# 10258392511/InverseProblemWithDiffusionModel

Measured on AMD Instinct MI355X. Metric: ALD reconstructions/sec (128x128 complex, R=40, 4-coil), higher is better.
Workload: dtype f32 (convolutions: operands as two fp16 pieces = 22 significand bits + 2 signs, three fp16 MFMAs per product, fp32 accumulate; every image scaled into fp16's range by an exact power of two from its producer's per-image maxima: any fp32 input, DESIGN.md 4.2); 1 GPU; ACDC-style 128x128 complex SENSE R=40 4-coil ALD reconstruction, NCSNv2Deepest ngf=128 (94.1M params, seeded random init), sigma 348->0.01 x 2311 levels x 3 steps, L2Penalty, denoise; 14 posterior samples = 14 on rank 0 + 13 per further rank (the 105-sample / 8-GPU partition of BASELINE config 3); samples_total=14, samples_this_rank=14, parallelism=sample-sharded x1, hip_graph=True, state_finite=True

## Files before the change

include/ipdm.h:

```cpp
#ifndef IPDM_H
#define IPDM_H

#include <stddef.h>
#include <stdint.h>

#ifdef __cplusplus
extern "C" {
#endif

#define IPDM_OK 0
#define IPDM_EINVAL (-1)
#define IPDM_EUNSUPPORTED (-2)

#define IPDM_ACT_NONE 0
#define IPDM_ACT_ELU 1
#define IPDM_ACT_RELU 2
#define IPDM_ACT_LRELU02 3
#define IPDM_ACT_SWISH 4
#define IPDM_ACT_COPY 5

#define IPDM_AMAX_WAYS 8
#define IPDM_AMAX_SLOT 128

#define IPDM_ABI_VERSION 4
// ... 192 lines not shown

int ipdm_philox_normal_f32(float* out, uint64_t seed, int64_t sample_offset, int64_t step_id, int plane,
                           int64_t n_samples, int64_t sample_elems, void* stream);

int ipdm_philox_block_host(uint64_t seed, int64_t sample, int64_t step_id, int plane, uint32_t quad, uint32_t* out4);


int ipdm_instnorm_plus_coef_f32(const float* x, const float* alpha, const float* gamma, const float* beta,
                                float* coef, int B, int C, int HW,
                                float* amax_bound ,
                                void* stream);
int ipdm_cond_instnorm_plus_coef_f32(const float* x, const float* embed, const int64_t* labels, int num_classes, int bias,
                                     float* coef, int B, int C, int HW, float* amax_bound, void* stream);
int ipdm_affine_act_f32(const float* x, const float* coef, float* y, int B, int C, int HW, int act, void* stream);
int ipdm_act_f32(const float* x, float* y, int64_t n, int act, void* stream);
int ipdm_scale_shift_f32(const float* x, float* y, int64_t n, float a, float b, void* stream);
int ipdm_add_f32(const float* x, const float* y, float* out, int64_t n, void* stream);
int ipdm_div_sigma_f32(const float* x, const float* sigmas, const int64_t* labels, float* out,
                       int B, int64_t sample_elems, void* stream);
int ipdm_conv3x3_thin_supported(int Cin, int Cout, int H, int W);
int ipdm_conv3x3_thin_f32(const float* x, const float* w, const float* bias,
                          const float* coef ,
                          float* out, int B, int Cin, int Cout, int H, int W, void* stream);
int ipdm_maxpool5_f32(const float* x, float* y, int planes, int H, int W, void* stream);
int ipdm_affine_avgpool5_f32(const float* x, const float* coef, float* y, int planes, int H, int W, void* stream);
int ipdm_meanpool2_f32(const float* x, float* y, int planes, int H, int W, void* stream);
int ipdm_bilinear_f32(const float* x, float* out, int planes, int in_h, int in_w, int out_h, int out_w,
                      int accumulate, int act ,
                      int planes_per_image, float* amax_out ,
                      void* stream);
int ipdm_trilinear_f32(const float* x, float* out, int planes, int in_d, int in_h, int in_w, int out_d, int out_h,
                       int out_w, int accumulate, int act, int planes_per_image, float* amax_out, void* stream);

int ipdm_groupnorm_coef_f32(const float* x, const float* weight, const float* bias, float* coef,
                            int B, int C, int HW, int G, float eps,
                            float* plane_amax ,
                            void* stream);
int ipdm_groupnorm_coef_partials_f32(const float* part1, int C1, const float* part2, int C2, int P, const float* weight,
                                     const float* bias, float* coef , int B, int G, float eps, void* stream);
int ipdm_groupnorm_coef_cat_f32(const float* x1, int C1, const float* x2, int C2, const float* weight, const float* bias,
                                float* coef, int B, int HW, int G, float eps, float* plane_amax ,
                                void* stream);
int ipdm_affine_act_cat_f32(const float* x1, int C1, const float* x2, int C2, const float* coef, float* y, int B, int HW,
                            int act, void* stream);
int ipdm_linear_f32(const float* x, const float* W, const float* bias, float* y, int B, int In, int Out,
                    int act, void* stream);
// ... 165 lines not shown
```

inverseproblemwithdiffusionmodel_amd/_lib.py:

```python
import ctypes
import os

import torch
from ctypes import c_char_p, c_double, c_float, c_int, c_int64, c_uint64, c_void_p


class ConvExt(ctypes.Structure):
    _fields_ = [("in_amax", c_void_p), ("bias_bstride", c_int), ("out_scale", c_float), ("res_second", c_int),
                ("out_amax", c_void_p), ("act_amax", c_void_p)]


_HERE = os.path.dirname(os.path.abspath(__file__))
LIB_PATH = os.environ.get("IPDM_LIB") or os.path.join(_HERE, "libipdm.so")

P = c_void_p

SIGNATURES = {
    "ipdm_abi_version": [],
    "ipdm_build_arch": [],
    "ipdm_upfirdn2d_f32": [P, P, P] + [c_int] * 14 + [P],
    "ipdm_fused_bias_act_f32": [P, P, P, P, c_int64, c_int, c_int, c_int, c_int, c_float, c_float, P],
    "ipdm_upfirdn2d_f16": [P, P, P] + [c_int] * 14 + [P],
    "ipdm_upfirdn2d_f64": [P, P, P] + [c_int] * 14 + [P],
    "ipdm_fused_bias_act_f16": [P, P, P, P, c_int64, c_int, c_int, c_int, c_int, c_float, c_float, P],
# ... 54 lines not shown
    "ipdm_espirit_kernels_c64": [P, c_int, c_int, c_int, c_double, P, P, P, P, P, P, c_int, c_int, c_int, c_int, P],
    "ipdm_espirit_pixel_c64": [P, P, c_int, c_float, c_int, P, P, c_int, c_int, c_int, c_int, P],
    "ipdm_espirit_c64": [P, c_int, c_int, c_int, c_double, c_float, c_int, P, P, P, P, P, P, P, c_int, c_int, c_int, c_int, P],
    "ipdm_kspace_tavg_c64": [P, P, c_int, P, P, c_int, c_int, c_int, c_int, c_int, P],
    "ipdm_singlecoil_prox_f32": [P, P, P, P, c_int, c_float, c_int, P, P, P, c_int, c_int, c_int, P],
    "ipdm_ald_singlecoil_step_f32": [P, P, P, P, P, P, c_float, c_float, c_uint64, c_int64, c_int64, P,
                                     P, P, c_int, c_float, c_int, P, c_int, c_int, c_int, P],
    "ipdm_langevin_step_f32": [P, P, P, c_float, c_float, c_uint64, c_int64, c_int64, P, c_int64, c_int64, P],
    "ipdm_philox_normal_f32": [P, c_uint64, c_int64, c_int64, c_int, c_int64, c_int64, P],
    "ipdm_philox_block_host": [c_uint64, c_int64, c_int64, c_int, ctypes.c_uint32, P],
    "ipdm_instnorm_plus_coef_f32": [P, P, P, P, P, c_int, c_int, c_int, P, P],
    "ipdm_cond_instnorm_plus_coef_f32": [P, P, P, c_int, c_int, P, c_int, c_int, c_int, P, P],
    "ipdm_affine_act_f32": [P, P, P, c_int, c_int, c_int, c_int, P],
    "ipdm_act_f32": [P, P, c_int64, c_int, P],
    "ipdm_scale_shift_f32": [P, P, c_int64, c_float, c_float, P],
    "ipdm_add_f32": [P, P, P, c_int64, P],
    "ipdm_div_sigma_f32": [P, P, P, P, c_int, c_int64, P],
    "ipdm_maxpool5_f32": [P, P, c_int, c_int, c_int, P],
    "ipdm_affine_avgpool5_f32": [P, P, P, c_int, c_int, c_int, P],
    "ipdm_meanpool2_f32": [P, P, c_int, c_int, c_int, P],
    "ipdm_bilinear_f32": [P, P, c_int, c_int, c_int, c_int, c_int, c_int, c_int, c_int, P, P],
    "ipdm_conv3x3_thin_supported": [c_int, c_int, c_int, c_int],
    "ipdm_conv3x3_thin_f32": [P, P, P, P, P, c_int, c_int, c_int, c_int, c_int, P],
    "ipdm_trilinear_f32": [P, P, c_int, c_int, c_int, c_int, c_int, c_int, c_int, c_int, c_int, c_int, P, P],
    "ipdm_groupnorm_coef_f32": [P, P, P, P, c_int, c_int, c_int, c_int, c_float, P, P],
    "ipdm_groupnorm_coef_partials_f32": [P, c_int, P, c_int, c_int, P, P, P, c_int, c_int, c_float, P],
    "ipdm_groupnorm_coef_cat_f32": [P, c_int, P, c_int, P, P, P, c_int, c_int, c_int, c_float, P, P],
    "ipdm_affine_act_cat_f32": [P, c_int, P, c_int, P, P, c_int, c_int, c_int, P],
    "ipdm_linear_f32": [P, P, P, P, c_int, c_int, c_int, c_int, P],
    "ipdm_attention_f32": [P, P, P, P, c_int, c_int, c_int, c_float, P],
    "ipdm_axpby_f32": [P, P, P, c_int64, c_float, c_float, P],
    "ipdm_sample_axpy2_f32": [P, P, P, P, P, P, c_int, c_int64, P],
    "ipdm_sample_norm_f32": [P, P, c_int, c_int64, P],
    "ipdm_conv_pack_weight_f32": [P, P, c_int, c_int, c_int, P],
    "ipdm_conv2d_f32": [P, P, P, P, c_int, P, P, P, c_int] + [c_int] * 8 + [P],
    "ipdm_conv_wino_weight_f32": [P, P, c_int, c_int, P],
    "ipdm_conv2d_wino_supported": [c_int, c_int, c_int, c_int, c_int],
    "ipdm_conv2d_wino_f32": [P, P, P, P, P, P, c_int, c_int, c_int, c_int, c_int, c_int, c_int, P],
    "ipdm_debug_set_stamp_buffer": [P],
    "ipdm_debug_lds_optin_count": [],
    "ipdm_conv3d_f32": [P, P, P, P, c_int, P, P, P, c_int] + [c_int] * 8 + [P],
    "ipdm_maxpool3d5_f32": [P, P, c_int, c_int, c_int, c_int, P],
    "ipdm_temporal_taps_f32": [P, P, c_int, c_int, c_int, c_int, c_int, P],
    "ipdm_conv_bx3_weight_bytes": [c_int, c_int, c_int],
    "ipdm_conv_bx3_pack_weight": [P, P, c_int, c_int, c_int, P],
    "ipdm_conv2d_bx3_f32": [P, P, P, P, c_int, P, P, P, c_int] + [c_int] * 7 + [P, P],
# ... 105 lines not shown
```

inverseproblemwithdiffusionmodel_amd/csrc/conv_thin.hip:

```cpp
#include "ipdm_common.h"

namespace {

template <int CIN>
__global__ __launch_bounds__(256) void conv3x3_fewin_kernel(const float* __restrict__ x, const float* __restrict__ w,
                                                            const float* __restrict__ bias, const float* __restrict__ coef,
                                                            float* __restrict__ out, int B, int Cout, int H, int W,
                                                            int co_blk) {
  const int Q = W >> 2;
  const long long items = (long long)B * H * Q;
  const int co0 = blockIdx.y * co_blk;
  const int co1 = min(Cout, co0 + co_blk);
  for (long long it = (long long)blockIdx.x * 256 + threadIdx.x; it < items; it += (long long)gridDim.x * 256) {
    const int q = (int)(it % Q);
    const long long t = it / Q;
    const int y = (int)(t % H);
    const int b = (int)(t / H);
    float in[CIN][3][6];
#pragma unroll
    for (int ci = 0; ci < CIN; ++ci) {
      float c0 = 0.f, c1 = 1.f, c2 = 0.f;
      if (coef) {
        const float* cf = coef + ((long long)b * CIN + ci) * 3;
        c0 = cf[0]; c1 = cf[1]; c2 = cf[2];
      }
#pragma unroll
      for (int r = 0; r < 3; ++r) {
        const int yy = y + r - 1;
        const bool row_ok = yy >= 0 && yy < H;
        const float* rp = x + (((long long)b * CIN + ci) * H + (row_ok ? yy : 0)) * W + 4 * q;
        const float4 m = *reinterpret_cast<const float4*>(rp);
        const float l = rp[q > 0 ? -1 : 0], rr = rp[q < Q - 1 ? 4 : 3];
        in[ci][r][0] = (row_ok && q > 0) ? (l - c0) * c1 + c2 : 0.f;
        in[ci][r][1] = row_ok ? (m.x - c0) * c1 + c2 : 0.f;
        in[ci][r][2] = row_ok ? (m.y - c0) * c1 + c2 : 0.f;
        in[ci][r][3] = row_ok ? (m.z - c0) * c1 + c2 : 0.f;
        in[ci][r][4] = row_ok ? (m.w - c0) * c1 + c2 : 0.f;
        in[ci][r][5] = (row_ok && q < Q - 1) ? (rr - c0) * c1 + c2 : 0.f;
      }
    }
    float* op = out + (((long long)b * Cout + co0) * H + y) * W + 4 * q;
    for (int co = co0; co < co1; ++co, op += (long long)H * W) {
      const float* wp = w + (long long)co * CIN * 9;
      const float bv = bias ? bias[co] : 0.f;
      float a0 = bv, a1 = bv, a2 = bv, a3 = bv;
#pragma unroll
      for (int ci = 0; ci < CIN; ++ci)
#pragma unroll
        for (int r = 0; r < 3; ++r)
#pragma unroll
          for (int c = 0; c < 3; ++c) {
            const float wv = wp[(ci * 3 + r) * 3 + c];
            a0 = fmaf(wv, in[ci][r][c], a0);
            a1 = fmaf(wv, in[ci][r][c + 1], a1);
            a2 = fmaf(wv, in[ci][r][c + 2], a2);
            a3 = fmaf(wv, in[ci][r][c + 3], a3);
          }
      *reinterpret_cast<float4*>(op) = make_float4(a0, a1, a2, a3);
    }
  }
}

template <int COUT, bool SHFL>
__global__ __launch_bounds__(256) void conv3x3_fewout_kernel(const float* __restrict__ x, const float* __restrict__ w,
                                                             const float* __restrict__ bias, float* __restrict__ out,
                                                             int B, int Cin, int H, int W) {
  __shared__ float red[3][COUT][4][64];
  const int Q = W >> 2;
  const long long items = (long long)B * H * Q;
  const long long HW = (long long)H * W;
  const int lane = threadIdx.x & 63, grp = threadIdx.x >> 6;
  for (long long it0 = (long long)blockIdx.x * 64; it0 < items; it0 += (long long)gridDim.x * 64) {
    const long long it = it0 + lane < items ? it0 + lane : items - 1;
    const bool live = it0 + lane < items;
    const int q = (int)(it % Q);
    const long long t = it / Q;
    const int y = (int)(t % H);
    const int b = (int)(t / H);
    float acc[COUT][3][4], hl[COUT][3], hr[COUT][3];
#pragma unroll
    for (int co = 0; co < COUT; ++co)
// ... 66 lines not shown
        for (int j = 0; j < 4; ++j) red[grp - 1][co][j][lane] = o[co][j];
    }
    __syncthreads();
    if (grp == 0 && live) {
#pragma unroll
      for (int co = 0; co < COUT; ++co) {
        const float bv = bias ? bias[co] : 0.f;
        float v[4];
#pragma unroll
        for (int j = 0; j < 4; ++j) v[j] = bv + (((o[co][j] + red[0][co][j][lane]) + red[1][co][j][lane]) + red[2][co][j][lane]);
        *reinterpret_cast<float4*>(out + (((long long)b * COUT + co) * H + y) * W + 4 * q) = make_float4(v[0], v[1], v[2], v[3]);
      }
    }
    __syncthreads();
  }
}

}

extern "C" int ipdm_conv3x3_thin_supported(int Cin, int Cout, int H, int W) {
  return (W % 4 == 0 && H > 0 && ((Cin >= 1 && Cin <= 3 && Cout >= 1) || (Cout >= 1 && Cout <= 3 && Cin >= 1))) ? 1 : 0;
}

extern "C" int ipdm_conv3x3_thin_f32(const float* x, const float* w, const float* bias, const float* coef, float* out, int B,
                                     int Cin, int Cout, int H, int W, void* stream) {
  IPDM_REQUIRE(B >= 0 && Cin > 0 && Cout > 0 && H > 0 && W > 0);
  if (!ipdm_conv3x3_thin_supported(Cin, Cout, H, W)) return IPDM_EUNSUPPORTED;
  if (B == 0) return IPDM_OK;
  IPDM_REQUIRE(x && w && out && x != out);
  if (((reinterpret_cast<uintptr_t>(x) | reinterpret_cast<uintptr_t>(out)) & 15) != 0) return IPDM_EUNSUPPORTED;
  hipStream_t s = ipdm_stream(stream);
  const long long items = (long long)B * H * (W / 4);
  const int gx = ipdm_ew_grid(items, 256);
  if (Cin <= 3 && Cin <= Cout) {
    int co_blk = Cout;
    while (co_blk > 8 && (long long)gx * ((Cout + co_blk - 1) / co_blk) < 2048) co_blk = (co_blk + 1) / 2;
    const dim3 grid(gx, (Cout + co_blk - 1) / co_blk);
    if (Cin == 1) hipLaunchKernelGGL(conv3x3_fewin_kernel<1>, grid, dim3(256), 0, s, x, w, bias, coef, out, B, Cout, H, W, co_blk);
    else if (Cin == 2) hipLaunchKernelGGL(conv3x3_fewin_kernel<2>, grid, dim3(256), 0, s, x, w, bias, coef, out, B, Cout, H, W, co_blk);
    else hipLaunchKernelGGL(conv3x3_fewin_kernel<3>, grid, dim3(256), 0, s, x, w, bias, coef, out, B, Cout, H, W, co_blk);
  } else {
    if (coef) return IPDM_EUNSUPPORTED;
    const int Q = W / 4;
    const int gx = ipdm_ew_grid(items, 64);
    const bool shfl = Q <= 64 && 64 % Q == 0;
#define IPDM_FEWOUT(CO)                                                                                                     \
  if (shfl) hipLaunchKernelGGL((conv3x3_fewout_kernel<CO, true>), dim3(gx), dim3(256), 0, s, x, w, bias, out, B, Cin, H, W); \
  else hipLaunchKernelGGL((conv3x3_fewout_kernel<CO, false>), dim3(gx), dim3(256), 0, s, x, w, bias, out, B, Cin, H, W)
    if (Cout == 1) { IPDM_FEWOUT(1); }
    else if (Cout == 2) { IPDM_FEWOUT(2); }
    else { IPDM_FEWOUT(3); }
#undef IPDM_FEWOUT
  }
  return ipdm_launch_status();
}
```

inverseproblemwithdiffusionmodel_amd/ncsn/models/layers.py:

```python
import os
from functools import partial

import torch
import torch.nn as nn

from ... import ops, _lib
from .normalization import InstanceNorm2dPlus, ConditionalInstanceNorm2dPlus, get_normalization


class _Act:

    def __init__(self, name):
        self.name = name
        self.code = ops.ACT_CODES[name]

    def __call__(self, x):
        return ops.act(x, self.code)


USE_WINOGRAD = os.environ.get("IPDM_WINOGRAD", "1") != "0"
FUSE_POOL = os.environ.get("IPDM_FUSE_POOL", "1") != "0"


def get_act(config):
# ... 32 lines not shown
        self._cache = ops.PackedWeightCache()

    def _cached(self, kind, build):
        return self._cache.get(self.weight, kind, build)

    def packed_wino(self):
        return self._cached("wino_f32", ops.conv_wino_weight)

    def packed_wino_bx3(self):
        return self._cached("wino_" + ops.CONV_IMPL, ops.conv_wino_split_weight)

    def packed_wino1d(self):
        return self._cached("wino1d", ops.conv_wino1d_weight)

    def route(self, x, site="ncsn", coef=None, **call):
        return ops.conv_route(site, self.ndim, self.kernel_size, self.dilation, self.in_planes, self.out_planes, tuple(x.shape[2:]),
                              x.data_ptr() % 16 == 0, ops.CONV_IMPL, winograd=USE_WINOGRAD, fuse_pool=FUSE_POOL,
                              full_range=self.full_range, coef=coef is not None,
                              coef_bound=getattr(coef, "_ipdm_amax_bound", None) is not None, **call)

    def fuses_input(self, x, coef):
        return self.route(x, coef=coef, act=ops.ACT_ELU) == ops.ROUTE_WINO1D

    def packed_conv1d(self):
        return self._cached("conv1d", ops.conv1d_weight)

    def packed_rows(self):
        if self.full_range and ops.CONV_IMPL == "hx2":
            return self._cached("rows_bx3", lambda w: ops.conv1d_rows_weight(w, impl="bx3"))
        return self._cached("rows_" + ops.CONV_IMPL, ops.conv1d_rows_weight)

    def conv1d_ok(self, x):
        return self.ndim == 1 and self.route(x) == ops.ROUTE_SEQ

    def packed(self):
        if self.full_range and ops.CONV_IMPL == "hx2":
            return self._cached("direct_bx3", lambda w: ops.conv_weight(w, impl="bx3"))
        return self._cached("direct_" + ops.CONV_IMPL, ops.conv_weight)

    def forward(self, x, coef=None, act=ops.ACT_NONE, residual=None, out=None, act_out=ops.ACT_NONE, raw=True,
                want_stats=False, in_amax=None, feeds_conv=True, res_second=False):
        bias = None if self.bias is None else self.bias.data
        dyn = ops.dynamic_range()
        produce = dyn and feeds_conv
        if in_amax is None and dyn and coef is None and act == ops.ACT_NONE:
            in_amax = ops.in_amax_for(x)
        if self.ndim == 1 and out is not None:
            raise NotImplementedError("Conv2d(ndim=1): no `out=` form")
        route = self.route(x, coef=coef, act=act, residual=residual is not None, out=out is not None, act_out=act_out, raw=raw,
                           want_stats=want_stats)
        tail = dict(act_out=act_out, raw=raw, in_amax=in_amax, want_amax=produce, res_second=res_second)
        if route == ops.ROUTE_SEQ:
            return ops.conv1d(x, self.packed_conv1d(), bias, residual, self.dilation, **tail)
        if route == ops.ROUTE_ROWS:
            return ops.conv1d_rows(x, self.packed_rows(), bias, coef, act, residual, self.dilation, **tail)
        if route == ops.ROUTE_WINO1D and coef is not None:
            return ops.conv2d_wino_bx3(x, self.packed_wino1d(), bias, residual, act_out=act_out, raw=raw, want_stats=want_stats,
                                       in_amax=getattr(coef, "_ipdm_amax_bound", None) if dyn else None, want_amax=produce,
                                       res_second=res_second, coef=coef, act=act)
        if route == ops.ROUTE_THIN:
            return ops.conv3x3_thin(x, self.weight.data, bias, coef)
        if route == ops.ROUTE_WINO_F32:
            return ops.conv2d_wino(x, self.packed_wino(), bias, residual, act_out=act_out, raw=raw,
                                   dilation=self.dilation)
        if route in (ops.ROUTE_WINO1D, ops.ROUTE_WINO_SPLIT):
            return ops.conv2d_wino_bx3(x, self.packed_wino1d() if route == ops.ROUTE_WINO1D else self.packed_wino_bx3(), bias, residual,
                                       act_out=act_out, raw=raw, dilation=self.dilation, want_stats=want_stats, in_amax=in_amax,
                                       want_amax=produce, res_second=res_second)
        if route == ops.ROUTE_WINO1D_VOL:
            return ops.conv3d(x, self._cached("wino1d_vol", ops.conv_wino1d_weight3d), bias, residual=residual, **tail)
        if route == ops.ROUTE_DIRECT3D:
            return ops.conv3d(x, self.packed(), bias, coef, act, residual, self.dilation, **tail)
        return ops.conv2d(x, self.packed(), bias, coef, act, residual, self.dilation, out=out, **tail)


def conv1x1(in_planes, out_planes, stride=1, bias=True, spec_norm=False, ndim=2):
    assert stride == 1 and not spec_norm
    return Conv2d(in_planes, out_planes, 1, bias=bias, ndim=ndim)


def conv3x3(in_planes, out_planes, stride=1, bias=True, spec_norm=False, ndim=2):
    assert stride == 1 and not spec_norm
    return Conv2d(in_planes, out_planes, 3, bias=bias, ndim=ndim)
# ... 72 lines not shown
                    x, out_act = self.convs[i](pooled, residual=x, act_out=code)
                else:
                    x = self.convs[i](pooled, residual=x)
            elif ops.split_impl():
                path, x = self.convs[i](pooled, residual=x, res_second=True, act_out=ops.ACT_COPY)
            else:
                path = self.convs[i](pooled)
                x = ops.add(path, x)
        return x, out_act


class RCUBlock(nn.Module):
    def __init__(self, features, n_blocks, n_stages, act=None, spec_norm=False, ndim=2):
        super().__init__()
        for i in range(n_blocks):
            for j in range(n_stages):
                setattr(self, '{}_{}_conv'.format(i + 1, j + 1), conv3x3(features, features, bias=False,
                                                                         spec_norm=spec_norm, ndim=ndim))
        self.stride = 1
        self.n_blocks = n_blocks
        self.n_stages = n_stages
        self.act = act

    def forward(self, x, x_act=None, want_act=False, feeds_conv=True):
        code = _act_code(self.act)
        for i in range(self.n_blocks):
            residual = x
            a = x_act if x_act is not None else ops.act(x, code)
            for j in range(self.n_stages):
                conv = getattr(self, '{}_{}_conv'.format(i + 1, j + 1))
                if j < self.n_stages - 1:
                    _, a = conv(a, act_out=code, raw=False)
                elif i < self.n_blocks - 1 or want_act:
                    x, x_act = conv(a, residual=residual, act_out=code)
                else:
                    x, x_act = conv(a, residual=residual, feeds_conv=feeds_conv), None
        return x, x_act


class MSFBlock(nn.Module):
    def __init__(self, in_planes, features, spec_norm=False, ndim=2):
        super().__init__()
        assert isinstance(in_planes, (list, tuple))
        self.convs = nn.ModuleList([conv3x3(p, features, bias=True, spec_norm=spec_norm, ndim=ndim) for p in in_planes])
        self.features = features

    def forward(self, xs, shape, act_out=ops.ACT_NONE):
        shape = tuple(int(s) for s in shape)
        sums = None
        n = len(self.convs)
        for i, conv in enumerate(self.convs):
            last_act = act_out if i == n - 1 else ops.ACT_NONE
            if tuple(xs[i].shape[2:]) == shape:
                if last_act != ops.ACT_NONE:
                    _, sums = conv(xs[i], residual=sums, act_out=last_act, raw=False)
                else:
                    sums = conv(xs[i], residual=sums, feeds_conv=False)
# ... 1 lines not shown
                h = conv(xs[i], feeds_conv=False)
                resize = ops.trilinear if h.dim() == 5 else ops.bilinear
                size = shape
                if h.dim() == 3:
                    resize, size = ops.linear1d, shape[0]
                sums = resize(h, size, out=sums, accumulate=sums is not None, act=last_act,
                              want_amax=i == n - 1 and ops.dynamic_range())
        return sums


class RefineBlock(nn.Module):
    def __init__(self, in_planes, features, act=None, start=False, end=False, maxpool=True, spec_norm=False, ndim=2):
        super().__init__()
        assert isinstance(in_planes, (tuple, list))
        self.n_blocks = n_blocks = len(in_planes)
        self.adapt_convs = nn.ModuleList([RCUBlock(in_planes[i], 2, 2, act, spec_norm=spec_norm, ndim=ndim)
                                          for i in range(n_blocks)])
        self.output_convs = RCUBlock(features, 3 if end else 1, 2, act, spec_norm=spec_norm, ndim=ndim)
        if not start:
            self.msf = MSFBlock(in_planes, features, spec_norm=spec_norm, ndim=ndim)
        self.crp = CRPBlock(features, 2, act, maxpool=maxpool, spec_norm=spec_norm, ndim=ndim)
        self.act = act

    def forward(self, xs, output_shape, xs_act=None, want_act=False, feeds_conv=None):
        assert isinstance(xs, (tuple, list))
        code = _act_code(self.act)
        xs_act = [None] * len(xs) if xs_act is None else xs_act
        single = self.n_blocks == 1
        hs = [self.adapt_convs[i](xs[i], xs_act[i], want_act=single) for i in range(len(xs))]
        if single:
            h, h_act = self.crp(hs[0][0], hs[0][1], want_act=True)
        else:
            a = self.msf([h[0] for h in hs], output_shape, act_out=code)
            h, h_act = self.crp(None, a, want_act=True)
        out, out_act = self.output_convs(h, h_act, want_act=want_act, feeds_conv=want_act if feeds_conv is None else feeds_conv)
        return (out, out_act) if want_act else out


class ResidualBlock(nn.Module):
    def __init__(self, input_dim, output_dim, resample=None, act=None, normalization=InstanceNorm2dPlus,
                 adjust_padding=False, dilation=None, spec_norm=False, ndim=2):
        super().__init__()
        conv3x3_ = partial(conv3x3, ndim=ndim)
        conv1x1_ = partial(conv1x1, ndim=ndim)
        dilated_conv3x3_ = partial(dilated_conv3x3, ndim=ndim)
        ConvMeanPool_ = partial(ConvMeanPool, ndim=ndim)
        self.non_linearity = act
        self.input_dim = input_dim
        self.output_dim = output_dim
        self.resample = resample
        self.normalization = normalization
        if resample == 'down':
            if dilation is not None:
                self.conv1 = dilated_conv3x3_(input_dim, input_dim, dilation=dilation, spec_norm=spec_norm)
                self.normalize2 = normalization(input_dim)
                self.conv2 = dilated_conv3x3_(input_dim, output_dim, dilation=dilation, spec_norm=spec_norm)
                conv_shortcut = partial(dilated_conv3x3_, dilation=dilation, spec_norm=spec_norm)
            else:
# ... 236 lines not shown
```

inverseproblemwithdiffusionmodel_amd/ncsn/models/ncsnv2.py:

```python
import torch
import torch.nn as nn

from . import get_sigmas
from .layers import ResidualBlock, RefineBlock, Conv2d, get_act, get_normalization
from ... import ops


class _NCSNv2Base(nn.Module):
    def __init__(self, config):
        super().__init__()
        self.logit_transform = config.data.logit_transform
        self.rescaled = config.data.rescaled
        self.norm = get_normalization(config, conditional=False)
        self.ngf = config.model.ngf
        self.num_classes = config.model.num_classes
        self.act = get_act(config)
        self.register_buffer('sigmas', get_sigmas(config))
        self.config = config
        self._in_coef = {}

    def _compute_cond_module(self, module, x):
        n = len(module)
        for i, m in enumerate(module):
            x = m(x, want_act=(i == n - 1))
        return x

    def _stage(self, cin, cout, resample=None, dilation=None):
        kw = dict(act=self.act, normalization=self.norm)
        if dilation is not None:
            kw["dilation"] = dilation
        return nn.ModuleList([ResidualBlock(cin, cout, resample=resample, **kw),
                              ResidualBlock(cout, cout, resample=None, **kw)])

    def _begin(self, x):
        if not x.is_cuda:
            raise RuntimeError("score network: expected GPU tensors (no CPU fallback in this build)")
        x = x.contiguous().float()
        if not self.logit_transform and not self.rescaled:
            key = (x.shape[0], x.shape[1], str(x.device))
            if key not in self._in_coef:
                self._in_coef[key] = torch.tensor([0.5, 2.0, 0.0], device=x.device).repeat(x.shape[0], x.shape[1], 1)
            return self.begin_conv(x, self._in_coef[key])
        return self.begin_conv(x)

    def _end(self, output, x, y):
        output = self.end_conv(self.normalizer(output, self.act.code))
        sig = self.sigmas if self.sigmas.dtype == torch.float32 else self.sigmas.to(torch.float32)
        return ops.div_sigma(output, sig, y.to(torch.int64))

    @staticmethod
    def _refine(block, pairs, shape, want_act=True):
        return block([p[0] for p in pairs], shape, [p[1] for p in pairs], want_act=want_act)


class NCSNv2Deepest(_NCSNv2Base):
    def __init__(self, config):
        super().__init__(config)
        ngf, ch = self.ngf, config.data.channels
        self.begin_conv = Conv2d(ch, ngf, 3, full_range=True)
        self.normalizer = self.norm(ngf)
        self.end_conv = Conv2d(ngf, ch, 3)
        self.res1 = self._stage(ngf, ngf)
        self.res2 = self._stage(ngf, 2 * ngf, 'down')
        self.res3 = self._stage(2 * ngf, 2 * ngf, 'down')
        self.res31 = self._stage(2 * ngf, 2 * ngf, 'down')
        self.res4 = self._stage(2 * ngf, 4 * ngf, 'down', dilation=2)
        self.res5 = self._stage(4 * ngf, 4 * ngf, 'down', dilation=4)
        self.refine1 = RefineBlock([4 * ngf], 4 * ngf, act=self.act, start=True)
        self.refine2 = RefineBlock([4 * ngf, 4 * ngf], 2 * ngf, act=self.act)
        self.refine3 = RefineBlock([2 * ngf, 2 * ngf], 2 * ngf, act=self.act)
        self.refine31 = RefineBlock([2 * ngf, 2 * ngf], 2 * ngf, act=self.act)
        self.refine4 = RefineBlock([2 * ngf, 2 * ngf], ngf, act=self.act)
        self.refine5 = RefineBlock([ngf, ngf], ngf, act=self.act, end=True)

# ... 90 lines not shown
```

inverseproblemwithdiffusionmodel_amd/ops.py:

```python
import ctypes
import os

import torch

from . import _lib
from ._lib import call, P

ACT_NONE, ACT_ELU, ACT_RELU, ACT_LRELU02, ACT_SWISH = 0, 1, 2, 3, 4
ACT_COPY = 5
CONV_TRACE = None

ACT_CODES = {"none": ACT_NONE, None: ACT_NONE, "elu": ACT_ELU, "relu": ACT_RELU, "lrelu": ACT_LRELU02,
             "swish": ACT_SWISH}


def _gpu(t, dtype=None, name="tensor"):
    if not isinstance(t, torch.Tensor) or not t.is_cuda:
        raise RuntimeError(f"ipdm: {name} must be a GPU tensor (the HIP path has no CPU fallback); got "
                           f"{getattr(t, 'device', type(t))}")
    if dtype is not None and t.dtype != dtype:
        raise TypeError(f"ipdm: {name} must be {dtype}, got {t.dtype}")
    return t if t.is_contiguous() else t.contiguous()


# ... 1491 lines not shown
    B, Cin, H, W = x.shape
    kk, Cin_w, Cout = wt.shape
    if Cin_w != Cin:
        raise ValueError(f"conv2d: weight Cin {Cin_w} != input Cin {Cin}")
    k = {1: 1, 9: 3}[kk]
    oh, ow = (H // 2, W // 2) if pool2 else (H, W)
    out, out_act, _, _ = _conv_outputs(x, (B, Cout, oh, ow), raw, act_out, "conv2d", out)
    e0 = _trace_open()
    call("ipdm_conv2d_f32", _ptr(x), _ptr(wt), _ptr(bias), _ptr(coef), act, _ptr(residual), _ptr(out), _ptr(out_act),
         act_out, B, Cin, Cout, H, W, k, dilation, int(bool(pool2)), _stream())
    _written(out)
    return _conv_done(e0, out, out_act, B=B, Cin=Cin, Cout=Cout, H=H, W=W, k=k, dil=dilation, res=residual is not None)


USE_THIN_CONV = os.environ.get("IPDM_THIN_CONV", "1") != "0"


def conv3x3_thin_ok(Cin, Cout, H, W, x=None):
    if x is not None and x.data_ptr() % 16:
        return False
    return USE_THIN_CONV and bool(_lib.lib.ipdm_conv3x3_thin_supported(int(Cin), int(Cout), int(H), int(W)))


def conv3x3_thin(x, weight, bias=None, coef=None):
    x = _gpu(x, torch.float32, "x")
    weight = _gpu(weight, torch.float32, "weight")
    B, Cin, H, W = x.shape
    Cout = weight.shape[0]
    if tuple(weight.shape) != (Cout, Cin, 3, 3):
        raise ValueError(f"conv3x3_thin: weight {tuple(weight.shape)} does not match input channels {Cin}")
    out = torch.empty((B, Cout, H, W), dtype=torch.float32, device=x.device)
    e0 = _trace_open()
    if coef is not None:
        coef = _gpu(coef, torch.float32, "coef")
        if tuple(coef.shape) != (B, Cin, 3):
            raise ValueError(f"conv3x3_thin: coef {tuple(coef.shape)} != {(B, Cin, 3)}")
    call("ipdm_conv3x3_thin_f32", _ptr(x), _ptr(weight), _ptr(bias), _ptr(coef), _ptr(out), B, Cin, Cout, H, W, _stream())
    return _conv_done(e0, out, None, B=B, Cin=Cin, Cout=Cout, H=H, W=W, k=3, dil=1, res=False, thin=True)


CONV_IMPL = os.environ.get("IPDM_CONV_IMPL", "hx2")
SPLIT_IMPLS = ("hx2", "bx3")
if CONV_IMPL not in SPLIT_IMPLS + ("f32",):
    raise ValueError(f"IPDM_CONV_IMPL={CONV_IMPL!r}: expected 'hx2', 'bx3' or 'f32'")


def split_impl():
    return CONV_IMPL in SPLIT_IMPLS


def impl_unbounded():
    env = os.environ.get("IPDM_CONV_IMPL_UNBOUNDED")
    if env:
        if env not in SPLIT_IMPLS + ("f32",):
            raise ValueError(f"IPDM_CONV_IMPL_UNBOUNDED={env!r}")
        return env
    return CONV_IMPL


# ... 483 lines not shown
```

Baseline: 0.1246 reconstructions/s.

## Fuse norm stats into thin begin conv and norm+ELU into end conv

The thin few-input-channel begin conv gains a stats epilogue that writes per-wave mean/M2 partials, so the following instance norm can skip a separate reduction pass. A new few-output end-conv kernel applies the InstanceNorm++ affine and ELU on the fly while streaming the many-channel input, removing the materialised normalized tensor. The refine4 output conv is also asked to emit stats. These paths add code complexity and rely on downstream consumers picking up the attached partials, which are not visible here.

```diff
diff --git a/include/ipdm.h b/include/ipdm.h
--- a/include/ipdm.h
+++ b/include/ipdm.h
@@ -238,6 +238,12 @@
 int ipdm_conv3x3_thin_f32(const float* x, const float* w, const float* bias,
                           const float* coef ,
                           float* out, int B, int Cin, int Cout, int H, int W, void* stream);
+int ipdm_conv3x3_thin_stats_partials(int Cin, int Cout, int H, int W);
+int ipdm_conv3x3_thin_stats_f32(const float* x, const float* w, const float* bias, const float* coef, float* out, float* part,
+                                int B, int Cin, int Cout, int H, int W, void* stream);
+int ipdm_conv3x3_fewout_fin_supported(int Cin, int Cout, int H, int W);
+int ipdm_conv3x3_fewout_fin_f32(const float* x, const float* w, const float* bias, const float* coef, int act, float* out,
+                                int B, int Cin, int Cout, int H, int W, void* stream);
 int ipdm_maxpool5_f32(const float* x, float* y, int planes, int H, int W, void* stream);
 int ipdm_affine_avgpool5_f32(const float* x, const float* coef, float* y, int planes, int H, int W, void* stream);
 int ipdm_meanpool2_f32(const float* x, float* y, int planes, int H, int W, void* stream);
diff --git a/inverseproblemwithdiffusionmodel_amd/_lib.py b/inverseproblemwithdiffusionmodel_amd/_lib.py
--- a/inverseproblemwithdiffusionmodel_amd/_lib.py
+++ b/inverseproblemwithdiffusionmodel_amd/_lib.py
@@ -100,6 +100,10 @@
     "ipdm_bilinear_f32": [P, P, c_int, c_int, c_int, c_int, c_int, c_int, c_int, c_int, P, P],
     "ipdm_conv3x3_thin_supported": [c_int, c_int, c_int, c_int],
     "ipdm_conv3x3_thin_f32": [P, P, P, P, P, c_int, c_int, c_int, c_int, c_int, P],
+    "ipdm_conv3x3_thin_stats_partials": [c_int, c_int, c_int, c_int],
+    "ipdm_conv3x3_thin_stats_f32": [P, P, P, P, P, P, c_int, c_int, c_int, c_int, c_int, P],
+    "ipdm_conv3x3_fewout_fin_supported": [c_int, c_int, c_int, c_int],
+    "ipdm_conv3x3_fewout_fin_f32": [P, P, P, P, c_int, P, c_int, c_int, c_int, c_int, c_int, P],
     "ipdm_trilinear_f32": [P, P, c_int, c_int, c_int, c_int, c_int, c_int, c_int, c_int, c_int, c_int, P, P],
     "ipdm_groupnorm_coef_f32": [P, P, P, P, c_int, c_int, c_int, c_int, c_float, P, P],
     "ipdm_groupnorm_coef_partials_f32": [P, c_int, P, c_int, c_int, P, P, P, c_int, c_int, c_float, P],
diff --git a/inverseproblemwithdiffusionmodel_amd/csrc/conv_thin.hip b/inverseproblemwithdiffusionmodel_amd/csrc/conv_thin.hip
--- a/inverseproblemwithdiffusionmodel_amd/csrc/conv_thin.hip
+++ b/inverseproblemwithdiffusionmodel_amd/csrc/conv_thin.hip
@@ -2,20 +2,24 @@
 
 namespace {
 
-template <int CIN>
+template <int CIN, bool STATS>
 __global__ __launch_bounds__(256) void conv3x3_fewin_kernel(const float* __restrict__ x, const float* __restrict__ w,
                                                             const float* __restrict__ bias, const float* __restrict__ coef,
                                                             float* __restrict__ out, int B, int Cout, int H, int W,
-                                                            int co_blk) {
+                                                            int co_blk, float* __restrict__ part, int P) {
   const int Q = W >> 2;
-  const long long items = (long long)B * H * Q;
+  const int HQ = H * Q;
+  const long long per = STATS ? (long long)P * 64 : (long long)HQ;
+  const long long items = (long long)B * per;
   const int co0 = blockIdx.y * co_blk;
   const int co1 = min(Cout, co0 + co_blk);
   for (long long it = (long long)blockIdx.x * 256 + threadIdx.x; it < items; it += (long long)gridDim.x * 256) {
-    const int q = (int)(it % Q);
-    const long long t = it / Q;
-    const int y = (int)(t % H);
-    const int b = (int)(t / H);
+    const int b = (int)(it / per);
+    const int rit = (int)(it % per);
+    const bool live = !STATS || rit < HQ;
+    const int ric = live ? rit : HQ - 1;
+    const int q = ric % Q;
+    const int y = ric / Q;
     float in[CIN][3][6];
 #pragma unroll
     for (int ci = 0; ci < CIN; ++ci) {
@@ -56,7 +60,25 @@
             a2 = fmaf(wv, in[ci][r][c + 2], a2);
             a3 = fmaf(wv, in[ci][r][c + 3], a3);
           }
-      *reinterpret_cast<float4*>(op) = make_float4(a0, a1, a2, a3);
+      if (live) *reinterpret_cast<float4*>(op) = make_float4(a0, a1, a2, a3);
+      if constexpr (STATS) {
+        const int lane = threadIdx.x & 63;
+        const float K = __builtin_bit_cast(float, __builtin_amdgcn_readfirstlane(__builtin_bit_cast(int, a0)));
+        const float d0 = live ? a0 - K : 0.f, d1 = live ? a1 - K : 0.f, d2 = live ? a2 - K : 0.f, d3 = live ? a3 - K : 0.f;
+        const float s1 = (d0 + d1) + (d2 + d3), s2 = (d0 * d0 + d1 * d1) + (d2 * d2 + d3 * d3);
+        const bool odd = lane & 1;
+        float v = odd ? s2 : s1;
+        v += __shfl_xor(odd ? s1 : s2, 1, 64);
+#pragma unroll
+        for (int m = 2; m < 64; m <<= 1) v += __shfl_xor(v, m, 64);
+        const float t2 = __shfl(v, 1, 64);
+        const float cnt = 4.f * (float)__popcll(__ballot(live));
+        if (lane == 0) {
+          const float dm = v / cnt;
+          float* sp = part + (((size_t)b * Cout + co) * P + rit / 64) * 3;
+          sp[0] = cnt; sp[1] = K + dm; sp[2] = fmaxf(t2 - v * dm, 0.f);
+        }
+      }
     }
   }
 }
@@ -169,23 +191,29 @@
   return (W % 4 == 0 && H > 0 && ((Cin >= 1 && Cin <= 3 && Cout >= 1) || (Cout >= 1 && Cout <= 3 && Cin >= 1))) ? 1 : 0;
 }
 
-extern "C" int ipdm_conv3x3_thin_f32(const float* x, const float* w, const float* bias, const float* coef, float* out, int B,
-                                     int Cin, int Cout, int H, int W, void* stream) {
+static int thin_launch(const float* x, const float* w, const float* bias, const float* coef, float* out, float* part, int B,
+                       int Cin, int Cout, int H, int W, void* stream) {
   IPDM_REQUIRE(B >= 0 && Cin > 0 && Cout > 0 && H > 0 && W > 0);
   if (!ipdm_conv3x3_thin_supported(Cin, Cout, H, W)) return IPDM_EUNSUPPORTED;
+  if (part && !ipdm_conv3x3_thin_stats_partials(Cin, Cout, H, W)) return IPDM_EUNSUPPORTED;
   if (B == 0) return IPDM_OK;
   IPDM_REQUIRE(x && w && out && x != out);
   if (((reinterpret_cast<uintptr_t>(x) | reinterpret_cast<uintptr_t>(out)) & 15) != 0) return IPDM_EUNSUPPORTED;
   hipStream_t s = ipdm_stream(stream);
-  const long long items = (long long)B * H * (W / 4);
+  const int P = part ? ipdm_conv3x3_thin_stats_partials(Cin, Cout, H, W) : 0;
+  const long long items = part ? (long long)B * P * 64 : (long long)B * H * (W / 4);
   const int gx = ipdm_ew_grid(items, 256);
   if (Cin <= 3 && Cin <= Cout) {
     int co_blk = Cout;
     while (co_blk > 8 && (long long)gx * ((Cout + co_blk - 1) / co_blk) < 2048) co_blk = (co_blk + 1) / 2;
     const dim3 grid(gx, (Cout + co_blk - 1) / co_blk);
-    if (Cin == 1) hipLaunchKernelGGL(conv3x3_fewin_kernel<1>, grid, dim3(256), 0, s, x, w, bias, coef, out, B, Cout, H, W, co_blk);
-    else if (Cin == 2) hipLaunchKernelGGL(conv3x3_fewin_kernel<2>, grid, dim3(256), 0, s, x, w, bias, coef, out, B, Cout, H, W, co_blk);
-    else hipLaunchKernelGGL(conv3x3_fewin_kernel<3>, grid, dim3(256), 0, s, x, w, bias, coef, out, B, Cout, H, W, co_blk);
+#define IPDM_FEWIN(CI)                                                                                                        \
+  if (part) hipLaunchKernelGGL((conv3x3_fewin_kernel<CI, true>), grid, dim3(256), 0, s, x, w, bias, coef, out, B, Cout, H, W, co_blk, part, P); \
+  else hipLaunchKernelGGL((conv3x3_fewin_kernel<CI, false>), grid, dim3(256), 0, s, x, w, bias, coef, out, B, Cout, H, W, co_blk, part, P)
+    if (Cin == 1) { IPDM_FEWIN(1); }
+    else if (Cin == 2) { IPDM_FEWIN(2); }
+    else { IPDM_FEWIN(3); }
+#undef IPDM_FEWIN
   } else {
     if (coef) return IPDM_EUNSUPPORTED;
     const int Q = W / 4;
@@ -201,3 +229,19 @@
   }
   return ipdm_launch_status();
 }
+
+extern "C" int ipdm_conv3x3_thin_stats_partials(int Cin, int Cout, int H, int W) {
+  if (!ipdm_conv3x3_thin_supported(Cin, Cout, H, W) || !(Cin <= 3 && Cin <= Cout)) return 0;
+  return (int)(((long long)H * (W / 4) + 63) / 64);
+}
+
+extern "C" int ipdm_conv3x3_thin_f32(const float* x, const float* w, const float* bias, const float* coef, float* out, int B,
+                                     int Cin, int Cout, int H, int W, void* stream) {
+  return thin_launch(x, w, bias, coef, out, nullptr, B, Cin, Cout, H, W, stream);
+}
+
+extern "C" int ipdm_conv3x3_thin_stats_f32(const float* x, const float* w, const float* bias, const float* coef, float* out,
+                                           float* part, int B, int Cin, int Cout, int H, int W, void* stream) {
+  IPDM_REQUIRE(part);
+  return thin_launch(x, w, bias, coef, out, part, B, Cin, Cout, H, W, stream);
+}
diff --git a/inverseproblemwithdiffusionmodel_amd/csrc/fewout_fin.hip b/inverseproblemwithdiffusionmodel_amd/csrc/fewout_fin.hip
--- /dev/null
+++ b/inverseproblemwithdiffusionmodel_amd/csrc/fewout_fin.hip
@@ -0,0 +1,185 @@
+#include "ipdm_common.h"
+
+namespace {
+
+__device__ __forceinline__ float fin_elu(float v, float mu, float sc, float sh) {
+  return ipdm_act_t<IPDM_ACT_ELU>((v - mu) * sc + sh);
+}
+
+template <int COUT, int R, bool SHFL>
+__global__ __launch_bounds__(256) void conv3x3_fewout_fin_kernel(const float* __restrict__ x, const float* __restrict__ w,
+                                                                 const float* __restrict__ bias, const float* __restrict__ coef,
+                                                                 float* __restrict__ out, int B, int Cin, int H, int W) {
+  __shared__ float red[3][COUT][R][4][64];
+  const int Q = W >> 2, S = (H + R - 1) / R;
+  const long long items = (long long)B * S * Q;
+  const long long HW = (long long)H * W;
+  const int lane = threadIdx.x & 63, grp = threadIdx.x >> 6;
+  for (long long it0 = (long long)blockIdx.x * 64; it0 < items; it0 += (long long)gridDim.x * 64) {
+    const long long it = it0 + lane < items ? it0 + lane : items - 1;
+    const bool live = it0 + lane < items;
+    const int q = (int)(it % Q);
+    const long long t = it / Q;
+    const int y0 = (int)(t % S) * R;
+    const int b = (int)(t / S);
+    float acc[COUT][R][3][4], hl[COUT][R][3], hr[COUT][R][3];
+#pragma unroll
+    for (int co = 0; co < COUT; ++co)
+#pragma unroll
+      for (int k = 0; k < R; ++k)
+#pragma unroll
+        for (int r = 0; r < 3; ++r) {
+          hl[co][k][r] = 0.f; hr[co][k][r] = 0.f;
+#pragma unroll
+          for (int j = 0; j < 4; ++j) acc[co][k][r][j] = 0.f;
+        }
+    bool ok[R + 2];
+    int ro[R + 2];
+#pragma unroll
+    for (int i = 0; i < R + 2; ++i) {
+      const int yy = y0 - 1 + i;
+      ok[i] = yy >= 0 && yy < H;
+      ro[i] = (yy < 0 ? 0 : (yy < H ? yy : H - 1)) * W;
+    }
+    const bool lf = q > 0, rt = q < Q - 1;
+    const float* base = x + (long long)b * Cin * HW + 4 * q;
+    const float* cfb = coef + (long long)b * Cin * 3;
+
+    struct Rows {
+      float4 m[R + 2];
+      float l[R + 2], r[R + 2];
+      float mu, sc, sh;
+    };
+    auto load = [&](int ci, Rows& d) {
+      const float* cp = base + ci * HW;
+      d.mu = cfb[ci * 3]; d.sc = cfb[ci * 3 + 1]; d.sh = cfb[ci * 3 + 2];
+#pragma unroll
+      for (int i = 0; i < R + 2; ++i) {
+        const float* rp = cp + ro[i];
+        d.m[i] = *reinterpret_cast<const float4*>(rp);
+        if constexpr (!SHFL) {
+          d.l[i] = rp[lf ? -1 : 0];
+          d.r[i] = rp[rt ? 4 : 3];
+        }
+      }
+    };
+    auto compute = [&](int ci, const Rows& d) {
+#pragma unroll
+      for (int i = 0; i < R + 2; ++i) {
+        const float mx = fin_elu(d.m[i].x, d.mu, d.sc, d.sh), my = fin_elu(d.m[i].y, d.mu, d.sc, d.sh);
+        const float mz = fin_elu(d.m[i].z, d.mu, d.sc, d.sh), mw = fin_elu(d.m[i].w, d.mu, d.sc, d.sh);
+        float l, rr;
+        if constexpr (SHFL) {
+          l = __shfl_up(mw, 1, 64);
+          rr = __shfl_down(mx, 1, 64);
+        } else {
+          l = fin_elu(d.l[i], d.mu, d.sc, d.sh);
+          rr = fin_elu(d.r[i], d.mu, d.sc, d.sh);
+        }
+#pragma unroll
+        for (int co = 0; co < COUT; ++co) {
+          const float* wc = w + ((long long)co * Cin + ci) * 9;
+#pragma unroll
+          for (int r = 0; r < 3; ++r) {
+            const int k = i - r;
+            if (k < 0 || k >= R) continue;
+            const float w0 = wc[r * 3], w1 = wc[r * 3 + 1], w2 = wc[r * 3 + 2];
+            hl[co][k][r] = fmaf(w0, l, hl[co][k][r]);
+            acc[co][k][r][0] = fmaf(w1, mx, acc[co][k][r][0]);
+            acc[co][k][r][0] = fmaf(w2, my, acc[co][k][r][0]);
+            acc[co][k][r][1] = fmaf(w0, mx, acc[co][k][r][1]);
+            acc[co][k][r][1] = fmaf(w1, my, acc[co][k][r][1]);
+            acc[co][k][r][1] = fmaf(w2, mz, acc[co][k][r][1]);
+            acc[co][k][r][2] = fmaf(w0, my, acc[co][k][r][2]);
+            acc[co][k][r][2] = fmaf(w1, mz, acc[co][k][r][2]);
+            acc[co][k][r][2] = fmaf(w2, mw, acc[co][k][r][2]);
+            acc[co][k][r][3] = fmaf(w0, mz, acc[co][k][r][3]);
+            acc[co][k][r][3] = fmaf(w1, mw, acc[co][k][r][3]);
+            hr[co][k][r] = fmaf(w2, rr, hr[co][k][r]);
+          }
+        }
+      }
+    };
+    for (int ci = grp; ci < Cin; ci += 8) {
+      Rows d0, d1;
+      const bool two = ci + 4 < Cin;
+      load(ci, d0);
+      if (two) load(ci + 4, d1);
+      compute(ci, d0);
+      if (two) compute(ci + 4, d1);
+    }
+    float o[COUT][R][4];
+#pragma unroll
+    for (int co = 0; co < COUT; ++co)
+#pragma unroll
+      for (int k = 0; k < R; ++k) {
+        const bool up = ok[k], dn = ok[k + 2];
+#pragma unroll
+        for (int j = 0; j < 4; ++j) {
+          float v = acc[co][k][1][j];
+          if (up) v += acc[co][k][0][j];
+          if (dn) v += acc[co][k][2][j];
+          o[co][k][j] = v;
+        }
+        float left = hl[co][k][1], right = hr[co][k][1];
+        if (up) { left += hl[co][k][0]; right += hr[co][k][0]; }
+        if (dn) { left += hl[co][k][2]; right += hr[co][k][2]; }
+        if (lf) o[co][k][0] += left;
+        if (rt) o[co][k][3] += right;
+      }
+    if (grp > 0) {
+#pragma unroll
+      for (int co = 0; co < COUT; ++co)
+#pragma unroll
+        for (int k = 0; k < R; ++k)
+#pragma unroll
+          for (int j = 0; j < 4; ++j) red[grp - 1][co][k][j][lane] = o[co][k][j];
+    }
+    __syncthreads();
+    if (grp == 0 && live) {
+#pragma unroll
+      for (int co = 0; co < COUT; ++co) {
+        const float bv = bias ? bias[co] : 0.f;
+#pragma unroll
+        for (int k = 0; k < R; ++k) {
+          if (y0 + k >= H) continue;
+          float v[4];
+#pragma unroll
+          for (int j = 0; j < 4; ++j)
+            v[j] = bv + (((o[co][k][j] + red[0][co][k][j][lane]) + red[1][co][k][j][lane]) + red[2][co][k][j][lane]);
+          *reinterpret_cast<float4*>(out + (((long long)b * COUT + co) * H + y0 + k) * W + 4 * q) = make_float4(v[0], v[1], v[2], v[3]);
+        }
+      }
+    }
+    __syncthreads();
+  }
+}
+
+}
+
+extern "C" int ipdm_conv3x3_fewout_fin_supported(int Cin, int Cout, int H, int W) {
+  return (W % 4 == 0 && H > 0 && Cout >= 1 && Cout <= 3 && Cin >= 1) ? 1 : 0;
+}
+
+extern "C" int ipdm_conv3x3_fewout_fin_f32(const float* x, const float* w, const float* bias, const float* coef, int act,
+                                           float* out, int B, int Cin, int Cout, int H, int W, void* stream) {
+  IPDM_REQUIRE(B >= 0 && Cin > 0 && Cout > 0 && H > 0 && W > 0);
+  if (!ipdm_conv3x3_fewout_fin_supported(Cin, Cout, H, W) || act != IPDM_ACT_ELU) return IPDM_EUNSUPPORTED;
+  if (B == 0) return IPDM_OK;
+  IPDM_REQUIRE(x && w && coef && out && x != out);
+  if (((reinterpret_cast<uintptr_t>(x) | reinterpret_cast<uintptr_t>(out)) & 15) != 0) return IPDM_EUNSUPPORTED;
+  hipStream_t s = ipdm_stream(stream);
+  const int Q = W / 4;
+  const bool shfl = Q <= 64 && 64 % Q == 0;
+#define IPDM_FEWOUT_FIN(CO, R)                                                                                              \
+  do {                                                                                                                      \
+    const int gx = ipdm_ew_grid((long long)B * ((H + R - 1) / R) * Q, 64);                                                  \
+    if (shfl) hipLaunchKernelGGL((conv3x3_fewout_fin_kernel<CO, R, true>), dim3(gx), dim3(256), 0, s, x, w, bias, coef, out, B, Cin, H, W); \
+    else hipLaunchKernelGGL((conv3x3_fewout_fin_kernel<CO, R, false>), dim3(gx), dim3(256), 0, s, x, w, bias, coef, out, B, Cin, H, W);     \
+  } while (0)
+  if (Cout == 1) IPDM_FEWOUT_FIN(1, 4);
+  else if (Cout == 2) IPDM_FEWOUT_FIN(2, 2);
+  else IPDM_FEWOUT_FIN(3, 2);
+#undef IPDM_FEWOUT_FIN
+  return ipdm_launch_status();
+}
diff --git a/inverseproblemwithdiffusionmodel_amd/ncsn/models/layers.py b/inverseproblemwithdiffusionmodel_amd/ncsn/models/layers.py
--- a/inverseproblemwithdiffusionmodel_amd/ncsn/models/layers.py
+++ b/inverseproblemwithdiffusionmodel_amd/ncsn/models/layers.py
@@ -78,6 +78,13 @@
     def fuses_input(self, x, coef):
         return self.route(x, coef=coef, act=ops.ACT_ELU) == ops.ROUTE_WINO1D
 
+    def streams_norm_input(self, x, act):
+        return (self.ndim == 2 and self.kernel_size == 3 and self.dilation == 1 and x.dim() == 4
+                and ops.conv3x3_fewout_fin_ok(self.in_planes, self.out_planes, x.shape[2], x.shape[3], x, act))
+
+    def stream_norm_input(self, x, coef, act):
+        return ops.conv3x3_fewout_fin(x, self.weight.data, None if self.bias is None else self.bias.data, coef, act)
+
     def packed_conv1d(self):
         return self._cached("conv1d", ops.conv1d_weight)
 
@@ -95,7 +102,7 @@
         return self._cached("direct_" + ops.CONV_IMPL, ops.conv_weight)
 
     def forward(self, x, coef=None, act=ops.ACT_NONE, residual=None, out=None, act_out=ops.ACT_NONE, raw=True,
-                want_stats=False, in_amax=None, feeds_conv=True, res_second=False):
+                want_stats=False, in_amax=None, feeds_conv=True, res_second=False, thin_stats=False):
         bias = None if self.bias is None else self.bias.data
         dyn = ops.dynamic_range()
         produce = dyn and feeds_conv
@@ -115,6 +122,8 @@
                                        in_amax=getattr(coef, "_ipdm_amax_bound", None) if dyn else None, want_amax=produce,
                                        res_second=res_second, coef=coef, act=act)
         if route == ops.ROUTE_THIN:
+            if thin_stats:
+                return ops.conv3x3_thin(x, self.weight.data, bias, coef, want_stats=True)
             return ops.conv3x3_thin(x, self.weight.data, bias, coef)
         if route == ops.ROUTE_WINO_F32:
             return ops.conv2d_wino(x, self.packed_wino(), bias, residual, act_out=act_out, raw=raw,
@@ -233,7 +242,7 @@
         self.n_stages = n_stages
         self.act = act
 
-    def forward(self, x, x_act=None, want_act=False, feeds_conv=True):
+    def forward(self, x, x_act=None, want_act=False, feeds_conv=True, want_stats=False):
         code = _act_code(self.act)
         for i in range(self.n_blocks):
             residual = x
@@ -244,6 +253,8 @@
                     _, a = conv(a, act_out=code, raw=False)
                 elif i < self.n_blocks - 1 or want_act:
                     x, x_act = conv(a, residual=residual, act_out=code)
+                elif want_stats:
+                    x, x_act = conv(a, residual=residual, feeds_conv=feeds_conv, want_stats=True), None
                 else:
                     x, x_act = conv(a, residual=residual, feeds_conv=feeds_conv), None
         return x, x_act
@@ -291,7 +302,7 @@
         self.crp = CRPBlock(features, 2, act, maxpool=maxpool, spec_norm=spec_norm, ndim=ndim)
         self.act = act
 
-    def forward(self, xs, output_shape, xs_act=None, want_act=False, feeds_conv=None):
+    def forward(self, xs, output_shape, xs_act=None, want_act=False, feeds_conv=None, want_stats=False):
         assert isinstance(xs, (tuple, list))
         code = _act_code(self.act)
         xs_act = [None] * len(xs) if xs_act is None else xs_act
@@ -302,7 +313,8 @@
         else:
             a = self.msf([h[0] for h in hs], output_shape, act_out=code)
             h, h_act = self.crp(None, a, want_act=True)
-        out, out_act = self.output_convs(h, h_act, want_act=want_act, feeds_conv=want_act if feeds_conv is None else feeds_conv)
+        out, out_act = self.output_convs(h, h_act, want_act=want_act, feeds_conv=want_act if feeds_conv is None else feeds_conv,
+                                         want_stats=want_stats and not want_act)
         return (out, out_act) if want_act else out
 
 
diff --git a/inverseproblemwithdiffusionmodel_amd/ncsn/models/ncsnv2.py b/inverseproblemwithdiffusionmodel_amd/ncsn/models/ncsnv2.py
--- a/inverseproblemwithdiffusionmodel_amd/ncsn/models/ncsnv2.py
+++ b/inverseproblemwithdiffusionmodel_amd/ncsn/models/ncsnv2.py
@@ -2,7 +2,7 @@
 import torch.nn as nn
 
 from . import get_sigmas
-from .layers import ResidualBlock, RefineBlock, Conv2d, get_act, get_normalization
+from .layers import ResidualBlock, RefineBlock, Conv2d, get_act, get_normalization, InstanceNorm2dPlus
 from ... import ops
 
 
@@ -40,16 +40,22 @@
             key = (x.shape[0], x.shape[1], str(x.device))
             if key not in self._in_coef:
                 self._in_coef[key] = torch.tensor([0.5, 2.0, 0.0], device=x.device).repeat(x.shape[0], x.shape[1], 1)
-            return self.begin_conv(x, self._in_coef[key])
-        return self.begin_conv(x)
+            return self.begin_conv(x, self._in_coef[key], thin_stats=ops.THIN_STATS)
+        return self.begin_conv(x, thin_stats=ops.THIN_STATS)
 
     def _end(self, output, x, y):
-        output = self.end_conv(self.normalizer(output, self.act.code))
+        code = self.act.code
+        if isinstance(self.normalizer, InstanceNorm2dPlus) and self.end_conv.streams_norm_input(output, code):
+            output = self.end_conv.stream_norm_input(output, self.normalizer.coef(output), code)
+        else:
+            output = self.end_conv(self.normalizer(output, code))
         sig = self.sigmas if self.sigmas.dtype == torch.float32 else self.sigmas.to(torch.float32)
         return ops.div_sigma(output, sig, y.to(torch.int64))
 
     @staticmethod
     def _refine(block, pairs, shape, want_act=True):
+        if not want_act and ops.END_STATS:
+            return block([p[0] for p in pairs], shape, [p[1] for p in pairs], want_act=False, want_stats=True)
         return block([p[0] for p in pairs], shape, [p[1] for p in pairs], want_act=want_act)
 
 
diff --git a/inverseproblemwithdiffusionmodel_amd/ops.py b/inverseproblemwithdiffusionmodel_amd/ops.py
--- a/inverseproblemwithdiffusionmodel_amd/ops.py
+++ b/inverseproblemwithdiffusionmodel_amd/ops.py
@@ -1537,7 +1537,38 @@
     return USE_THIN_CONV and bool(_lib.lib.ipdm_conv3x3_thin_supported(int(Cin), int(Cout), int(H), int(W)))
 
 
-def conv3x3_thin(x, weight, bias=None, coef=None):
+THIN_STATS = os.environ.get("IPDM_THIN_STATS", "1") != "0"
+THIN_FIN = os.environ.get("IPDM_THIN_FIN", "1") != "0"
+END_STATS = os.environ.get("IPDM_END_STATS", "1") != "0"
+
+
+def conv3x3_thin_stats_ok(Cin, Cout, H, W, x=None):
+    return (THIN_STATS and USE_STATS_EPILOGUE and conv3x3_thin_ok(Cin, Cout, H, W, x)
+            and int(_lib.lib.ipdm_conv3x3_thin_stats_partials(int(Cin), int(Cout), int(H), int(W))) > 0)
+
+
+def conv3x3_fewout_fin_ok(Cin, Cout, H, W, x, act=ACT_ELU):
+    return (THIN_FIN and act == ACT_ELU and x.dim() == 4 and Cout <= 3 < Cin and conv3x3_thin_ok(Cin, Cout, H, W, x)
+            and bool(_lib.lib.ipdm_conv3x3_fewout_fin_supported(int(Cin), int(Cout), int(H), int(W))))
+
+
+def conv3x3_fewout_fin(x, weight, bias, coef, act=ACT_ELU):
+    x = _gpu(x, torch.float32, "x")
+    weight = _gpu(weight, torch.float32, "weight")
+    coef = _gpu(coef, torch.float32, "coef")
+    B, Cin, H, W = x.shape
+    Cout = weight.shape[0]
+    if tuple(weight.shape) != (Cout, Cin, 3, 3):
+        raise ValueError(f"conv3x3_fewout_fin: weight {tuple(weight.shape)} does not match input channels {Cin}")
+    if tuple(coef.shape) != (B, Cin, 3):
+        raise ValueError(f"conv3x3_fewout_fin: coef {tuple(coef.shape)} != {(B, Cin, 3)}")
+    out = torch.empty((B, Cout, H, W), dtype=torch.float32, device=x.device)
+    e0 = _trace_open()
+    call("ipdm_conv3x3_fewout_fin_f32", _ptr(x), _ptr(weight), _ptr(bias), _ptr(coef), act, _ptr(out), B, Cin, Cout, H, W, _stream())
+    return _conv_done(e0, out, None, B=B, Cin=Cin, Cout=Cout, H=H, W=W, k=3, dil=1, res=False, thin=True, fin=True)
+
+
+def conv3x3_thin(x, weight, bias=None, coef=None, want_stats=False):
     x = _gpu(x, torch.float32, "x")
     weight = _gpu(weight, torch.float32, "weight")
     B, Cin, H, W = x.shape
@@ -1550,6 +1581,13 @@
         coef = _gpu(coef, torch.float32, "coef")
         if tuple(coef.shape) != (B, Cin, 3):
             raise ValueError(f"conv3x3_thin: coef {tuple(coef.shape)} != {(B, Cin, 3)}")
+    if want_stats and conv3x3_thin_stats_ok(Cin, Cout, H, W, x):
+        P = int(_lib.lib.ipdm_conv3x3_thin_stats_partials(Cin, Cout, H, W))
+        part = torch.empty((B, Cout, P, 3), dtype=torch.float32, device=x.device)
+        call("ipdm_conv3x3_thin_stats_f32", _ptr(x), _ptr(weight), _ptr(bias), _ptr(coef), _ptr(out), _ptr(part), B, Cin, Cout, H, W,
+             _stream())
+        out._ipdm_partials = (part, (out._version, out.data_ptr()))
+        return _conv_done(e0, out, None, B=B, Cin=Cin, Cout=Cout, H=H, W=W, k=3, dil=1, res=False, thin=True, stats=True)
     call("ipdm_conv3x3_thin_f32", _ptr(x), _ptr(weight), _ptr(bias), _ptr(coef), _ptr(out), B, Cin, Cout, H, W, _stream())
     return _conv_done(e0, out, None, B=B, Cin=Cin, Cout=Cout, H=H, W=W, k=3, dil=1, res=False, thin=True)
 
```

Result: faster. 0.1259 reconstructions/s (median of 6 runs) (+1.0%).
